# tiborcamargo/KinectPy

Hardware: AMD Instinct MI355X
Metric: Mpoints/sec end-to-end (unproject+filter+ICP), 4-sensor frame (higher is better)
Workload: dtype f64 decisions / f32 storage

## Files before the change

### kinectpy_amd/csrc/kpx_icpdefs.h

```cpp
#pragma once
#include <limits.h>

#include "kpx_internal.h"

namespace kpx {

typedef double d4 __attribute__((ext_vector_type(4)));
#ifndef KPX_ICP_WPE
#define KPX_ICP_WPE 3
#endif

#ifndef KPX_ICP_WAVES
#define KPX_ICP_WAVES 4
#endif
constexpr int kIWaves = KPX_ICP_WAVES;
constexpr int kIThreads = kIWaves * 64;
constexpr int kRT = 2;
constexpr int kWaves = 4;
constexpr int kRowsPerBlock = kWaves * kRT * 16;
constexpr int kCT = 32;
constexpr int kStageDoubles = kCT * 64;
#ifndef KPX_SEED_STRIDE
#define KPX_SEED_STRIDE 128
#endif
constexpr int kSeedStride = KPX_SEED_STRIDE;
constexpr double kSentinel = 1e300;
constexpr int kFRT = 4;
constexpr int kFRowsPerBlock = kWaves * kFRT * 16;
constexpr int kFCT = 64;
constexpr int kFStageFloats = kFCT * 64;
constexpr int kCand = 64;
constexpr int kAcc = 44;

struct IcpState {
    double T[16];
    double fitness, rmse;
    double count;
    int32_t iter, done;
    double motion, reach;
    double last_motion;
    double smax;
};
// ... 53 lines not shown
        int slot = 17;
#pragma unroll
        for (int a = 0; a < 6; ++a)
#pragma unroll
            for (int c = a; c < 6; ++c) put(slot++, J[a] * J[c]);
#pragma unroll
        for (int a = 0; a < 6; ++a) put(38 + a, J[a] * res);
    }
}
__host__ __device__ __forceinline__ unsigned long long progress_searched(unsigned long long searched, int64_t n)
{
    const unsigned long long cls = n > 0 ? (searched * 127ull + (unsigned long long)n - 1ull) / (unsigned long long)n : 0ull;
    return (cls > 127ull ? 127ull : cls) << 33;
}
constexpr int kSearchedWord = 8;
__device__ __forceinline__ unsigned long long searched_take(unsigned long long *ticket, int lane_in_block)
{
    unsigned long long v = 0ull;
    if (lane_in_block < 8) {
        v = __hip_atomic_load(ticket + kSearchedWord + lane_in_block, __ATOMIC_RELAXED, __HIP_MEMORY_SCOPE_AGENT);
        __hip_atomic_store(ticket + kSearchedWord + lane_in_block, 0ull, __ATOMIC_RELAXED, __HIP_MEMORY_SCOPE_AGENT);
    }
    if (lane_in_block < 64) {
        unsigned lo = (unsigned)v, hi = (unsigned)(v >> 32);
#pragma unroll
        for (int o = 1; o < 8; o <<= 1) {
            const unsigned ol = (unsigned)__shfl_xor((int)lo, o, 64), oh = (unsigned)__shfl_xor((int)hi, o, 64);
            const unsigned long long sum = (((unsigned long long)hi << 32) | lo) + (((unsigned long long)oh << 32) | ol);
            lo = (unsigned)sum; hi = (unsigned)(sum >> 32);
        }
        v = ((unsigned long long)hi << 32) | lo;
    }
    return v;
}
__device__ __forceinline__ double tile_tree16(const double *x)
{
    double a[8];
#pragma unroll
    for (int i = 0; i < 8; ++i) a[i] = x[2 * i] + x[2 * i + 1];
    return ((a[0] + a[1]) + (a[2] + a[3])) + ((a[4] + a[5]) + (a[6] + a[7]));
}
typedef unsigned u2 __attribute__((ext_vector_type(2)));
__device__ __forceinline__ unsigned hi32(double v) { return __builtin_bit_cast(u2, v)[1]; }

struct RobustLoss {
    int32_t kind;
    double k;
    __device__ __forceinline__ double weight(double r) const
    {
        switch (kind) {
        case KPX_LOSS_L1: return 1.0 / fabs(r);
        case KPX_LOSS_HUBER: return k / fmax(fabs(r), k);
        case KPX_LOSS_CAUCHY: { const double q = r / k; return 1.0 / (1.0 + q * q); }
        case KPX_LOSS_GM: { const double d = k + r * r; return k / (d * d); }
        case KPX_LOSS_TUKEY: { const double q = fmin(1.0, fabs(r) / k); const double u = 1.0 - q * q; return u * u; }
        default: return 1.0;
        }
    }
};
__device__ __forceinline__ void robust_row(const RobustLoss &loss, const double J[6], double r, double *acc)
{
    const double w = loss.weight(r);
    if (!isfinite(w)) return;
    double wJ[6];
#pragma unroll
    for (int p = 0; p < 6; ++p) wJ[p] = w * J[p];
    int q = 17;
#pragma unroll
    for (int p = 0; p < 6; ++p)
#pragma unroll
        for (int c = p; c < 6; ++c) acc[q++] += wJ[p] * J[c];
#pragma unroll
    for (int p = 0; p < 6; ++p) acc[38 + p] += wJ[p] * r;
// ... 82 lines not shown
```

### kinectpy_amd/csrc/kpx_icpiter.h

```cpp
#pragma once
#include "kpx_icpdefs.h"
#include "kpx_fixed.h"
#include "kpx_icpsolve.h"
#include "kpx_nnlocal.h"

namespace kpx {

constexpr int kIRows = kIWaves * kLRows;
constexpr int kCertHist = 64;
constexpr int kChainRec = 32;
constexpr int kChainRecords = 64;
constexpr int kChainWords = 24;
constexpr unsigned long long kChainEmpty = 0xFFF8C0DEC0DEC0DEull;
constexpr int kAccSet = kAccCopies * kAcc * kFixedWords;
constexpr int kStampBlocks = 4096;
__device__ unsigned long long g_icp_stamp[kStampBlocks][8];
__device__ unsigned long long g_icp_wave[kStampBlocks * 4][4];
__device__ unsigned long long g_cert_check[8];
__device__ unsigned long long g_chain_stamp[64][48];
__device__ __forceinline__ void chain_tick(unsigned long long *row, int slot, bool on)
{
    if (row && on) row[slot] = wall_clock64();
}
__device__ __forceinline__ void phase_tick(unsigned long long *__restrict__ armed, int slot, unsigned bid)
// ... 55 lines not shown
    if (first && g_cert_check[2] == 0ull) {
        g_cert_check[3] = (unsigned long long)k; g_cert_check[4] = __builtin_bit_cast(unsigned long long, st->last_motion);
        g_cert_check[5] = __builtin_bit_cast(unsigned long long, st->motion); g_cert_check[6] = __builtin_bit_cast(unsigned long long, c_skin);
    }
    atomicAdd(&g_cert_check[0], (unsigned long long)certified);
    atomicAdd(&g_cert_check[1], (unsigned long long)searched);
}
__device__ __forceinline__ IcpFuse ticket_fuse(const IcpProblem &P, int max_iter, double rel_fit, double rel_rmse, unsigned long long tag, int light,
                                               CertPolicy pol, double *chain_rec, unsigned long long *stamp)
{
    return IcpFuse{ (IcpState *)nullptr, P.ring, max_iter, rel_fit, rel_rmse, P.result, P.progress, tag, P.ring + kAccSet,
                    (light & 1) ? P.light_key : (double *)nullptr, P.sbbox, (light & 2) ? P.cert : (uint32_t *)nullptr,
                    (light & 2) ? P.thist : (double *)nullptr, (light & 4) ? 1 : 0, pol, chain_rec, stamp };
}
template <int THREADS, bool SEARCHED>
__device__ __forceinline__ unsigned long long winner_take(unsigned long long *acc, unsigned long long *ticket, int nacc, double *s_sums, int tix_w)
{
    if (tix_w < kAcc) s_sums[tix_w] = tix_w < nacc ? fixed_total_coherent(acc, tix_w) : 0.0;
    const unsigned long long n_searched = SEARCHED ? searched_take(ticket, tix_w) : 0ull;
    if (THREADS > 64) __syncthreads(); else wave_lds_fence();
    for (int e = tix_w; e < kAccSet; e += THREADS) __hip_atomic_store(acc + e, 0ull, __ATOMIC_RELAXED, __HIP_MEMORY_SCOPE_AGENT);
    if (tix_w == 0) __hip_atomic_store(ticket, 0ull, __ATOMIC_RELAXED, __HIP_MEMORY_SCOPE_AGENT);
    return n_searched;
}
__device__ __forceinline__ void winner_publish(IcpState *st, const IcpState *work, double *thist, int k, unsigned long long *progress, unsigned long long tag,
                                               unsigned long long n_searched, int64_t n, int lane)
{
    if (lane < (int)(sizeof(IcpState) / sizeof(double))) reinterpret_cast<double *>(st)[lane] = reinterpret_cast<const double *>(work)[lane];
    if (thist && k + 1 < kCertHist && lane < 12) thist[12 * (k + 1) + lane] = work->T[lane];
    if (lane == 0 && progress)
        __hip_atomic_store(progress, tag | progress_searched(n_searched, n) | ((unsigned long long)(work->done ? 1 : 0) << 32) | (unsigned long long)(unsigned)(k + 1),
                           __ATOMIC_RELAXED, __HIP_MEMORY_SCOPE_SYSTEM);
}

template <bool PERSIST = false>
__device__ __forceinline__ void icp_iter_body(const unsigned bid, const unsigned nblocks, const float *__restrict__ src, int64_t n, const float *__restrict__ tgt,
                                                       const float *__restrict__ tn, const double *__restrict__ Bs,
                                                       const int32_t *__restrict__ orig, const float *__restrict__ tile_box,
                                                       const float *__restrict__ group_box, int32_t n_groups,
                                                       const double *__restrict__ tbbox, const int32_t *__restrict__ row_of,
                                                       const float *__restrict__ src_sorted, int32_t *__restrict__ idx_sorted,
                                                       float *__restrict__ ptgt_sorted,
                                                       int32_t *__restrict__ idx_cur, double *__restrict__ d2_cur, double max_d2, int mode,
                                                       int k, const IcpState *__restrict__ st, unsigned long long *acc,
                                                       unsigned long long *__restrict__ tile_visits, IcpFuse fuse)
{
    const unsigned tix = PERSIST ? (unsigned)opaque_i((int)threadIdx.x) : threadIdx.x;
    __shared__ IcpState s_state;
    __shared__ double s_sums[kAcc];
    __shared__ float rowk[kIWaves][16][8];
    __shared__ float rowsrc[kIWaves][16][3];
    __shared__ uint32_t rowc[kIWaves][16];
    __shared__ int32_t rowi[kIWaves][16][2];
    __shared__ double s_key;
    const int wave = PERSIST ? __builtin_amdgcn_readfirstlane((int)(tix >> 6)) : (int)(tix >> 6), lane = tix & 63, q = lane >> 4, j = lane & 15;
    const int64_t row_base = ((int64_t)bid * kIWaves + wave) * kLRows;
    const int64_t last = n - 1;
    const unsigned long long t_block_start = (tile_visits && tix == 0) ? wall_clock64() : 0ull;
    const double t2max = target_t2max(tbbox);
    float my_src[3] = { 0.0f, 0.0f, 0.0f }, my_pt[3] = { 0.0f, 0.0f, 0.0f }, my_nrm[3] = { 0.0f, 0.0f, 0.0f };
    int32_t my_row = 0, my_prev = -1;
    uint32_t my_cert = 0u;
    const bool certs = fuse.ticket && fuse.light_key && fuse.cert;
    if (PERSIST && k > 0) {
        if (lane < 16) {
            my_row = rowi[wave][lane][1];
#pragma unroll
            for (int a = 0; a < 3; ++a) { my_src[a] = rowsrc[wave][lane][a]; my_pt[a] = rowk[wave][lane][a]; my_nrm[a] = rowk[wave][lane][3 + a]; }
            my_prev = __float_as_int(rowk[wave][lane][6]);
            if (certs) my_cert = rowc[wave][lane];
        }
    } else if (lane < 16) {
        const int64_t r = row_base + lane < last ? row_base + lane : last;
        if (idx_cur || d2_cur) my_row = row_of[r];
#pragma unroll
        for (int a = 0; a < 3; ++a) my_src[a] = src_sorted[3 * r + a];
        if (PERSIST) {
#pragma unroll
            for (int a = 0; a < 3; ++a) rowsrc[wave][lane][a] = my_src[a];
            rowc[wave][lane] = 0u;
        }
        if (k > 0) {
            my_prev = idx_sorted[r];
#pragma unroll
            for (int a = 0; a < 3; ++a) my_pt[a] = ptgt_sorted[3 * r + a];
            if (certs) my_cert = fuse.cert[r];
        }
    }
    __shared__ double s_thist[kCertHist][12];
    if (PERSIST) {
        if (certs && k < kCertHist && tix < 12) s_thist[k][tix] = st->T[tix];
    } else if (certs && k > 0)
        for (int e = tix; e < 12 * (k < kCertHist ? k : kCertHist); e += kIThreads) (&s_thist[0][0])[e] = fuse.thist[e];
    GroupPre gpre;
    group_pre_load(gpre, group_box, n_groups, lane);
    if (!PERSIST && mode == 1 && k > 0 && lane < 16) {
        const float *np_ = tn + 3 * (int64_t)(my_prev > 0 ? my_prev : 0);
#pragma unroll
        for (int a = 0; a < 3; ++a) my_nrm[a] = np_[a];
    }
    const double *Tk = st->T;
    static_assert(sizeof(IcpState) % sizeof(double) == 0, "IcpState is copied as doubles");
    if (fuse.ticket && tix < sizeof(IcpState) / sizeof(double))
        reinterpret_cast<double *>(&s_state)[tix] = reinterpret_cast<const double *>(st)[tix];
    if (fuse.pair) {
        const IcpState *in = fuse.pair + ((k + 1) & 1);
        IcpState *out = fuse.pair + (k & 1);
        const unsigned long long *prev = fuse.ring + (int64_t)((k + 2) % 3) * kAccSet;
        if (k > 0 && tix < kAcc) s_sums[tix] = (int)tix < (mode == 1 ? kAcc : 17) ? fixed_total(prev, tix) : 0.0;
        if (tix == 0) s_state = *in;
        __syncthreads();
        if (s_state.done) {
            if (bid == 0 && tix == 0) *out = s_state;
            return;
        }
        __shared__ FinishScratch s_fs;
        if (k > 0 && wave == 0)
            icp_finish_wave(s_sums, n, mode, k - 1, fuse.max_iter, fuse.rel_fit, fuse.rel_rmse, &s_state, bid == 0 ? fuse.result : (double *)nullptr,
                            s_fs, lane);
        __syncthreads();
        if (bid == 0) {
            unsigned long long *next = fuse.ring + (int64_t)((k + 1) % 3) * kAccSet;
            for (int e = tix; e < kAccSet; e += kIThreads) next[e] = 0ull;
            if (tix == 0) {
                *out = s_state;
                if (k > 0 && fuse.progress)
                    __hip_atomic_store(fuse.progress, fuse.tag | ((unsigned long long)(s_state.done ? 1 : 0) << 32) | (unsigned long long)(unsigned)k,
                                       __ATOMIC_RELEASE, __HIP_MEMORY_SCOPE_SYSTEM);
            }
        }
        if (s_state.done) return;
        Tk = s_state.T;
        acc = fuse.ring + (int64_t)(k % 3) * kAccSet;
    } else if (st->done) return;
    bool skip = false;
    if (fuse.ticket && fuse.light_key) {
        const double key = PERSIST ? (k > 0 ? s_key : 0.0) : fuse.light_key[bid];
        skip = key > 0.0 && (st->motion + st->reach) * (1.0 + 1e-6) + 1e-6 < key;
    }
    __shared__ double s_light[kIWaves];
    const int nacc = mode == 1 ? kAcc : 17;
    if (tile_visits && tix == 0 && bid < kStampBlocks) { g_icp_stamp[bid][7] = skip ? 1ull : 0ull; g_icp_stamp[bid][6] = (unsigned long long)nblocks; }
    do {
    if (skip) break;
    __shared__ int32_t lists[kIWaves][kLScratch];
    __shared__ double rowd[kIWaves][16][kRowStride];
    __shared__ float rowf[kIWaves][16][kRowFStride];
    __shared__ double sh[kAcc][kIRows + 1];
    if (tile_visits && tix == 0 && bid < kStampBlocks) {
        g_icp_stamp[bid][0] = t_block_start;
        g_icp_stamp[bid][6] = (unsigned long long)nblocks;
    }
    phase_tick(tile_visits, 1, bid);
    if (certs && (k > 0 || PERSIST)) __syncthreads();
    if (PERSIST && fuse.stamp && tix == 0) {
        const unsigned long long t = wall_clock64();
        if (bid == 0) fuse.stamp[0] = t;
        atomicMax(&fuse.stamp[5], t);
        atomicMin(&fuse.stamp[10], t);
    }

    const double c_reach = certs ? st->reach : 0.0;
    const double c_skin = cert_skin(certs, k, st, max_d2, fuse.pol);
    bool my_active = true, my_certd = false;
    if (lane < 16) {
        const int64_t i = my_row;
        double s[3];
        xform_row(Tk, my_src, s);
        const double seed = row_seed(s);
        double bv = INFINITY;
        int32_t bj = INT_MAX;
        if (k > 0 && my_prev >= 0) { bv = partner_bound(s, seed, my_pt); bj = my_prev; }
        bound_clamp(seed, max_d2, t2max, bv, bj);
        double rb0 = bv - 1.0;
        if (certs) {
            const bool certd = cert_test(s, my_src, my_prev, my_pt, bj, my_cert, s_thist[my_cert & 63u], c_reach, c_skin, fuse.cert_check, rb0);
            my_active = (!certd || fuse.cert_check) && row_base + lane <= last;
            my_certd = certd && row_base + lane <= last;
        }
        rowd[wave][lane][0] = s[0]; rowd[wave][lane][1] = s[1]; rowd[wave][lane][2] = s[2];
        rowd[wave][lane][3] = rb0;
        rowd[wave][lane][4] = seed; rowd[wave][lane][5] = bv;
        rowi[wave][lane][0] = bj; rowi[wave][lane][1] = (int32_t)i;
#pragma unroll
        for (int a = 0; a < 3; ++a) { rowk[wave][lane][a] = my_pt[a]; rowk[wave][lane][3 + a] = my_nrm[a]; }
        rowk[wave][lane][6] = __int_as_float(my_prev);
    }
    if (PERSIST && fuse.stamp) {
        const bool searched = lane < 16 && my_active && !my_certd;
        const unsigned long long sm = __builtin_amdgcn_ballot_w64(searched);
        const unsigned long long np = __builtin_amdgcn_ballot_w64(searched && my_prev < 0);
        const unsigned long long nc = __builtin_amdgcn_ballot_w64(searched && (my_cert & ~63u) == 0u);
        if (lane == 0 && sm) {
            atomicAdd(&fuse.stamp[26], 1ull); atomicAdd(&fuse.stamp[27], (unsigned long long)__builtin_popcountll(sm));
            atomicAdd(&fuse.stamp[28], (unsigned long long)__builtin_popcountll(np)); atomicAdd(&fuse.stamp[29], (unsigned long long)__builtin_popcountll(nc));
        }
    }
    const unsigned act_mask = (unsigned)(__builtin_amdgcn_ballot_w64(lane < 16 && my_active) & 0xFFFFull);
    const unsigned certd_mask = (unsigned)(__builtin_amdgcn_ballot_w64(lane < 16 && my_certd) & 0xFFFFull);
    wave_lds_fence();
    WaveRows w;
    w.a = q < 3 ? rowd[wave][j][q] : 1.0;
    w.rows = &rowd[wave][0][0];
    w.rowsf = &rowf[wave][0][0];
#pragma unroll
    for (int r = 0; r < 4; ++r) {
        const int rr = q + 4 * r;
        w.seed[r] = rowd[wave][rr][4];
        w.best[r] = rowd[wave][rr][5];
        w.bcol[r] = rowi[wave][rr][0];
        w.rb0[r] = rowd[wave][rr][3];
    }
    w.skin = c_skin;
    w.act_mask = act_mask;
    w.light_gap2 = -1.0;
    w.dbg = (PERSIST && fuse.stamp && bid == 0 && wave == 0) ? fuse.stamp + 16 : (unsigned long long *)nullptr;
    phase_tick(tile_visits, 2, bid);
    if (PERSIST) chain_tick(fuse.stamp, 1, bid == 0 && tix == 0);
    const unsigned long long t_sweep = tile_visits ? wall_clock64() : 0ull;
    unsigned long long swept = 0ull;
    int lane_p = 0, wave_p = 0, q_p = 0, j_p = 0;
    int64_t row_base_p = 0;
    auto rederive = [&]() {
        lane_p = opaque_i((int)(threadIdx.x & 63)); wave_p = opaque_i((int)(threadIdx.x >> 6)); q_p = lane_p >> 4; j_p = lane_p & 15;
        row_base_p = ((int64_t)bid * kIWaves + wave_p) * kLRows;
    };
    if (act_mask != 0u) {
        wave_lds_fence();
        swept = sweep_wave<true, true, PERSIST>(w, Bs, orig, tile_box, group_box, n_groups, t2max, lists[wave], &gpre);
        rederive();
        if (certs && fuse.cert_check && j_p == 0) {
#pragma unroll
            for (int r = 0; r < 4; ++r) {
                const int rr = q_p + 4 * r;
                if (((certd_mask >> rr) & 1u) != 0u && w.bcol[r] != rowi[wave_p][rr][0])
                    cert_check_disagreement(k, row_base_p + rr, rowi[wave_p][rr][0], w.bcol[r], PERSIST ? rowc[wave_p][rr] : fuse.cert[row_base_p + rr]);
            }
        }
        if (certs && j_p == 0) {
#pragma unroll
            for (int r = 0; r < 4; ++r) {
                const int rr = q_p + 4 * r;
                if (((act_mask >> rr) & 1u) != 0u && ((certd_mask >> rr) & 1u) == 0u) {
                    const uint32_t cw = cert_word(w.sec[r], w.eps_out, w.rb_out[r], k);
                    if (PERSIST) rowc[wave_p][rr] = cw; else fuse.cert[row_base_p + rr] = cw;
                }
            }
        }
    }
    if (act_mask == 0u) rederive();
    __shared__ int s_cnt[kIWaves];
    if (lane_p == 0) s_cnt[wave_p] = __builtin_popcount(act_mask & ~certd_mask);
    const unsigned visited = (unsigned)(swept & 0xFFFFu);
    if (certs && fuse.cert_check && lane_p == 0)
        cert_check_count(bid == 0 && wave_p == 0, k, st, c_skin, __builtin_popcount(certd_mask), __builtin_popcount(act_mask & ~certd_mask));
    if (lane_p == 0) s_light[wave_p] = act_mask == 0xFFFFu ? w.light_gap2 : -1.0;
    if (tile_visits && lane_p == 0 && bid < kStampBlocks && kIWaves <= 4) {
        unsigned long long *o = g_icp_wave[bid * 4 + wave_p];
        int with = 0;
#pragma unroll
        for (int r = 0; r < 4; ++r) with += (w.bcol[r] >= 0 && w.bcol[r] != INT_MAX) ? 1 : 0;
        o[0] = t_sweep; o[1] = wall_clock64(); o[2] = swept; o[3] = (unsigned long long)with;
    }
    phase_tick(tile_visits, 3, bid);
    if (PERSIST) chain_tick(fuse.stamp, 2, bid == 0 && lane_p == 0 && wave_p == 0);
    if (PERSIST && fuse.stamp && bid == 0 && lane_p == 0 && wave_p == 0) { fuse.stamp[13] = swept; fuse.stamp[14] = (unsigned long long)act_mask | ((unsigned long long)certd_mask << 16); }
    if (tile_visits && lane_p == 0) atomicAdd(tile_visits + ((bid * kIWaves + wave_p) & (kVisitSlots - 1)), (unsigned long long)visited);
    wave_lds_fence();
    if (j_p == 0) {
#pragma unroll
        for (int r = 0; r < 4; ++r) rowi[wave_p][q_p + 4 * r][0] = w.bcol[r];
    }
    wave_lds_fence();

    const int lane_e = lane_p, wave_e = wave_p;
    if (lane_e < 16) {
        const int col = wave_e * 16 + lane_e;
        for (int a = 0; a < nacc; ++a) sh[a][col] = 0.0;
        if (row_base_p + lane_e <= last) {
            const int32_t bj = rowi[wave_e][lane_e][0];
            const int64_t i = rowi[wave_e][lane_e][1];
            const bool none = bj < 0 || bj == INT_MAX;
            const int32_t out_j = none ? -1 : bj;
            const int32_t prev_j = __float_as_int(rowk[wave_e][lane_e][6]);
            const bool changed = k == 0 || out_j != prev_j;
            if (idx_cur) idx_cur[i] = out_j;
            if (PERSIST) rowk[wave_e][lane_e][6] = __int_as_float(out_j);
            else if (changed) idx_sorted[row_base_p + lane_e] = out_j;
            if (none) {
                if (d2_cur) d2_cur[i] = INFINITY;
            } else {
                const double s[3] = { rowd[wave_e][lane_e][0], rowd[wave_e][lane_e][1], rowd[wave_e][lane_e][2] };
                float tf[3] = { rowk[wave_e][lane_e][0], rowk[wave_e][lane_e][1], rowk[wave_e][lane_e][2] }, nf[3] = { rowk[wave_e][lane_e][3], rowk[wave_e][lane_e][4], rowk[wave_e][lane_e][5] };
                if (changed) {
                    const float *tp = tgt + 3 * (int64_t)bj;
#pragma unroll
                    for (int c = 0; c < 3; ++c) tf[c] = tp[c];
                    if (mode == 1) {
                        const float *np_ = tn + 3 * (int64_t)bj;
#pragma unroll
                        for (int c = 0; c < 3; ++c) nf[c] = np_[c];
                    }
#pragma unroll
                    for (int c = 0; c < 3; ++c) {
                        if (PERSIST) { rowk[wave_e][lane_e][c] = tf[c]; rowk[wave_e][lane_e][3 + c] = nf[c]; }
                        else ptgt_sorted[3 * (row_base_p + lane_e) + c] = tf[c];
                    }
                }
                const double t[3] = { (double)tf[0], (double)tf[1], (double)tf[2] };
                const double d2 = pair_d2(s, t);
                if (d2_cur) d2_cur[i] = d2;
                if (d2 < max_d2) pair_terms(s, t, d2, mode == 1, nf, [&](int slot, double v) { sh[slot][col] = v; });
            }
        }
    }
    __syncthreads();
    phase_tick(tile_visits, 4, bid);
    const int tix_e = wave_e * 64 + lane_e;
    if (tix_e < nacc) {
        unsigned long long lo = 0ull, hi = 0ull;
#pragma unroll
        for (int t = 0; t < kIWaves; ++t) {
            unsigned long long l, h;
            fixed_split(tile_tree16(&sh[tix_e][16 * t]), l, h);
            fixed_accumulate(lo, hi, l, h);
        }
        unsigned long long *slot = acc + (((int64_t)(bid & (kAccCopies - 1)) * kAcc + tix_e) * kFixedWords);
        if (fuse.ticket) fixed_add_words_performed(slot, lo, hi); else fixed_add_words(slot, lo, hi);
    } else if (!PERSIST && fuse.ticket && tix_e == nacc) {
        int cnt = 0;
#pragma unroll
        for (int wv = 0; wv < kIWaves; ++wv) cnt += s_cnt[wv];
        if (cnt) {
            const unsigned long long back = __hip_atomic_fetch_add(fuse.ticket + kSearchedWord + (bid & 7u), (unsigned long long)cnt, __ATOMIC_RELAXED, __HIP_MEMORY_SCOPE_AGENT);
            asm volatile("" ::"v"(back));
        }
    }
    if (fuse.light_key && tix == kIThreads - 1) {
        double g2 = INFINITY;
        bool light = true;
#pragma unroll
        for (int wv = 0; wv < kIWaves; ++wv) { light = light && s_light[wv] >= 0.0; g2 = fmin(g2, s_light[wv]); }
        const double nk = light ? st->motion + sqrt(g2) * (1.0 - 1e-9) : 0.0;
        if (PERSIST) s_key = nk; else fuse.light_key[bid] = nk;
    }
    phase_tick(tile_visits, 5, bid);
    } while (false);
    if (PERSIST && fuse.stamp && tix == 0) {
        const unsigned long long t = wall_clock64();
        if (bid == 0) fuse.stamp[3] = t;
        atomicMax(&fuse.stamp[11], t);
    }
    if (!fuse.ticket) return;
    __shared__ unsigned s_ticket;
    __syncthreads();
    if (tix == 0) s_ticket = (unsigned)__hip_atomic_fetch_add(fuse.ticket, 1ull, __ATOMIC_RELAXED, __HIP_MEMORY_SCOPE_AGENT);
    __syncthreads();
// ... 16 lines not shown
    const double *tbbox_w = tbbox;
    asm volatile("" : "+s"(tbbox_w));
    const double t2max_w = target_t2max(tbbox_w);
    IcpState *stw = const_cast<IcpState *>(st);
    IcpState *work = &s_state;
    if (PERSIST)
        icp_finish_wave_call(s_sums, n, mode, k, fuse.max_iter, fuse.rel_fit, fuse.rel_rmse, work, (double *)nullptr, &s_tail, lane,
                             fuse.light_key ? fuse.sbbox : (const double *)nullptr, max_d2, t2max_w, fuse.stamp ? fuse.stamp + 32 : (unsigned long long *)nullptr);
    else
        icp_finish_wave(s_sums, n, mode, k, fuse.max_iter, fuse.rel_fit, fuse.rel_rmse, work, fuse.result, s_tail, lane,
                        LightSkip{ fuse.light_key ? fuse.sbbox : (const double *)nullptr, max_d2, t2max_w });
    wave_lds_fence();
    if (PERSIST) chain_tick(fuse.stamp, 8, lane == 0);
    if (PERSIST) {
        static_assert(sizeof(IcpState) == kChainWords * sizeof(double), "record layout");
        __syncthreads();
        if (lane < kChainWords)
            __hip_atomic_store(reinterpret_cast<unsigned long long *>(fuse.chain_rec + (size_t)kChainRec * (k + 1)) + lane,
                               reinterpret_cast<const unsigned long long *>(&s_state)[lane], __ATOMIC_RELAXED, __HIP_MEMORY_SCOPE_AGENT);
        if (work->done && fuse.result) {
            if (lane < 16) fuse.result[lane] = work->T[lane];
            if (lane == 0) { fuse.result[16] = work->fitness; fuse.result[17] = work->rmse; fuse.result[18] = (double)k; fuse.result[19] = work->count; }
        }
        if (lane == 0 && fuse.progress && work->done)
            __hip_atomic_store(fuse.progress, fuse.tag | (1ull << 32) | (unsigned long long)(unsigned)(k + 1), __ATOMIC_RELAXED, __HIP_MEMORY_SCOPE_SYSTEM);
        chain_tick(fuse.stamp, 9, lane == 0);
        if (fuse.stamp && lane == 0) fuse.stamp[12] = __builtin_amdgcn_s_memtime();
        return;
    }
    winner_publish(stw, work, fuse.cert ? fuse.thist : (double *)nullptr, k, fuse.progress, fuse.tag, n_searched, n, lane);
}


__global__ __launch_bounds__(kIThreads) __attribute__((amdgpu_waves_per_eu(KPX_ICP_WPE, KPX_ICP_WPE))) void icp_iter_kernel(const float *__restrict__ src, int64_t n, const float *__restrict__ tgt,
                                                       const float *__restrict__ tn, const double *__restrict__ Bs,
                                                       const int32_t *__restrict__ orig, const float *__restrict__ tile_box,
                                                       const float *__restrict__ group_box, int32_t n_groups,
                                                       const double *__restrict__ tbbox, const int32_t *__restrict__ row_of,
                                                       const float *__restrict__ src_sorted, int32_t *__restrict__ idx_sorted,
                                                       float *__restrict__ ptgt_sorted,
                                                       int32_t *__restrict__ idx_cur, double *__restrict__ d2_cur, double max_d2, int mode,
                                                       int k, const IcpState *__restrict__ st, unsigned long long *acc,
                                                       unsigned long long *__restrict__ tile_visits, IcpFuse fuse)
{
    icp_iter_body(blockIdx.x, gridDim.x, src, n, tgt, tn, Bs, orig, tile_box, group_box, n_groups, tbbox, row_of, src_sorted, idx_sorted, ptgt_sorted,
                  idx_cur, d2_cur, max_d2, mode, k, st, acc, tile_visits, fuse);
}

__global__ __launch_bounds__(kIThreads) __attribute__((amdgpu_waves_per_eu(KPX_ICP_WPE, KPX_ICP_WPE))) void icp_iter_batch_kernel(IcpBatchArgs args, double max_d2, int mode, int max_iter, double rel_fit,
                                                       double rel_rmse, unsigned long long *__restrict__ tile_visits, int light, CertPolicy pol)
{
    const IcpProblem &P = args.p[batch_problem(args)];
    const unsigned bid = blockIdx.x - P.block0;
    const float *__restrict__ tgt = P.tgt, *__restrict__ tn = P.tn, *__restrict__ tile_box = P.tile_box, *__restrict__ group_box = P.group_box;
    const double *__restrict__ Bs = P.Bs, *__restrict__ tbbox = P.tbbox;
    const int32_t *__restrict__ orig = P.orig;
    const int32_t n_groups = P.n_groups;
    const int k = P.k;
    const IcpFuse fuse = ticket_fuse(P, max_iter, rel_fit, rel_rmse, P.tag, light, pol, nullptr, nullptr);
    icp_iter_body(bid, P.blocks, P.src, P.n, tgt, tn, Bs, orig, tile_box, group_box, n_groups, tbbox, P.row_of, P.src_sorted, P.idx_sorted, P.ptgt_sorted,
                  P.idx_cur, P.d2_cur, max_d2, mode, k, P.pair, P.ring, tile_visits, fuse);
}

__global__ __launch_bounds__(kIThreads) __attribute__((amdgpu_waves_per_eu(KPX_ICP_WPE, KPX_ICP_WPE))) void icp_chain_kernel(IcpBatchArgs args, const float *__restrict__ tgt,
                                                       const float *__restrict__ tn, const double *__restrict__ Bs,
                                                       const int32_t *__restrict__ orig, const float *__restrict__ tile_box,
                                                       const float *__restrict__ group_box, int32_t n_groups,
                                                       const double *__restrict__ tbbox, double max_d2, int mode, int max_iter, double rel_fit,
                                                       double rel_rmse, unsigned long long tag, unsigned long long *__restrict__ tile_visits, int light,
                                                       CertPolicy pol, unsigned long long limit_ticks, unsigned long long *abort_word)
{
    const int pi = batch_problem(args);
    const IcpProblem &P = args.p[pi];
    const unsigned bid = blockIdx.x - P.block0;
    __shared__ IcpState s_cur;
    __shared__ int s_abort;
    const unsigned long long t0 = wall_clock64();
    if (threadIdx.x == 0) s_abort = 0;
    __syncthreads();
    for (int k = 0; k <= max_iter; ++k) {
        asm volatile("" : "+s"(tgt), "+s"(tn), "+s"(Bs), "+s"(orig), "+s"(tile_box), "+s"(group_box), "+s"(tbbox));
        asm volatile("" : "+s"(max_d2), "+s"(mode), "+s"(n_groups), "+s"(pol.calm), "+s"(pol.factor), "+s"(pol.smin), "+s"(pol.smax));
// ... 57 lines not shown
```

### kinectpy_amd/csrc/kpx_icprows.h

```cpp
#pragma once
#include "kpx_icpiter.h"

namespace kpx {

constexpr int kRowsBlock = 64;
static_assert(kRowsBlock == kIRows, "IcpProblem::block0 / blocks count 64-row blocks for icp_iter_batch_kernel and icp_rows_kernel alike");

constexpr int kDppXor1 = 0xB1, kDppXor2 = 0x4E, kDppHalfMirror = 0x141, kDppMirror = 0x140;
__device__ __forceinline__ double row16_tree_sum(double v)
{
    v += dpp_f64<kDppXor1>(v);
    v += dpp_f64<kDppXor2>(v);
    v += dpp_f64<kDppHalfMirror>(v);
    v += dpp_f64<kDppMirror>(v);
    return v;
}

template <int MODE>
__global__ __launch_bounds__(64) __attribute__((amdgpu_waves_per_eu(KPX_ICP_WPE, KPX_ICP_WPE))) void icp_rows_kernel(IcpBatchArgs args, double max_d2, int max_iter, double rel_fit,
                                                                                                                     double rel_rmse, unsigned long long *__restrict__ tile_visits,
                                                                                                                     int light, CertPolicy pol)
{
    constexpr int NACC = MODE == 1 ? kAcc : 17;
    const IcpProblem P = args.p[batch_problem(args)];
    const unsigned bid = blockIdx.x - P.block0;
    const int k = P.k;
    IcpState *const st = P.pair;
    if (st->done) return;

    __shared__ IcpState s_state;
    __shared__ double s_sums[kAcc];
    __shared__ FinishScratch s_tail;
    __shared__ double rowd[kRowsBlock][kRowStride];
    __shared__ float rowf[kLRows][kRowFStride];
    __shared__ float rowk[kRowsBlock][11];
    __shared__ int32_t rowi[kRowsBlock];
    __shared__ uint32_t rowc[kRowsBlock];
    __shared__ int32_t rowm[kRowsBlock];
    __shared__ int32_t lists[kLScratch];
    static_assert(kLScratch * sizeof(int32_t) >= 4 * kAcc * sizeof(double), "the tile partials reuse the sweep's scratch");
    double (*s_part)[kAcc] = reinterpret_cast<double (*)[kAcc]>(lists);

    const int lane = threadIdx.x;
    const unsigned long long lt = (1ull << lane) - 1ull;
    const int64_t last = P.n - 1;
    const int64_t row = (int64_t)bid * kRowsBlock + lane;
    const bool valid = lane < kRowsBlock && row <= last;
    const int64_t r = valid ? row : last;
    const bool certs = (light & 2) != 0, use_light = (light & 1) != 0, cert_check = (light & 4) != 0;
// ... 217 lines not shown
```

### kinectpy_amd/csrc/kpx_nnlocal.h

```cpp
#pragma once
#include "kpx_icpdefs.h"
#include "kpx_morton.h"

namespace kpx {

constexpr int kLGroupTiles = 16;
constexpr int kLRows = 16;
constexpr int kLList = 320;
constexpr int kVisitSlots = 1024;

__global__ __launch_bounds__(256) void nn_local_prep_kernel(const float *__restrict__ tgt, int64_t m, double *__restrict__ Bs,
                                                            int32_t *__restrict__ orig, float *__restrict__ tile_box,
                                                            float *__restrict__ group_box)
{
    const int64_t j = (int64_t)blockIdx.x * 256 + threadIdx.x;
    double b0 = 0.0, b1 = 0.0, b2 = 0.0, b3 = kSentinel;
    float lo[3] = { kBoxBig, kBoxBig, kBoxBig }, hi[3] = { -kBoxBig, -kBoxBig, -kBoxBig };
    if (j < m) {
        const int64_t o = orig[j];
        const float fx = tgt[3 * o], fy = tgt[3 * o + 1], fz = tgt[3 * o + 2];
        const double tx = fx, ty = fy, tz = fz;
        b0 = -2.0 * tx; b1 = -2.0 * ty; b2 = -2.0 * tz;
        b3 = fma(tx, tx, fma(ty, ty, tz * tz));
        lo[0] = hi[0] = fx; lo[1] = hi[1] = fy; lo[2] = hi[2] = fz;
// ... 43 lines not shown
    if (r >= n) return;
    const int64_t i = row_of[r];
    double s[3];
    xform_row(T, src + 3 * i, s);
    const double seed = row_seed(s);
    reinterpret_cast<double2 *>(A64)[2 * r] = make_double2(s[0], s[1]);
    reinterpret_cast<double2 *>(A64)[2 * r + 1] = make_double2(s[2], 1.0);
    K64[r] = seed;
    double bv = INFINITY;
    int32_t bj = INT_MAX;
    if (prev) {
        const int32_t j = prev[i];
        if (j >= 0 && j != INT_MAX) { bv = partner_bound(s, seed, tgt + 3 * (int64_t)j); bj = j; }
    }
    if (max_d2 > 0.0) bound_clamp(seed, max_d2, target_t2max(tbbox), bv, bj);
    init_val[r] = bv;
    init_idx[r] = bj;
}

__device__ __forceinline__ unsigned fold16(unsigned long long m) { return (unsigned)((m | (m >> 16) | (m >> 32) | (m >> 48)) & 0xFFFFull); }

template <int CTRL>
__device__ __forceinline__ int dpp_i32(int v) { return __builtin_amdgcn_update_dpp(v, v, CTRL, 0xF, 0xF, false); }
template <int CTRL>
__device__ __forceinline__ double dpp_f64(double v)
{
    typedef int i2 __attribute__((ext_vector_type(2)));
    i2 b = __builtin_bit_cast(i2, v);
    b[0] = dpp_i32<CTRL>(b[0]);
    b[1] = dpp_i32<CTRL>(b[1]);
    return __builtin_bit_cast(double, b);
}
constexpr int kRor1 = 0x121, kRor2 = 0x122, kRor4 = 0x124, kRor8 = 0x128;
__device__ __forceinline__ double row16_all_max(double v)
{
    v = fmax(v, dpp_f64<kRor1>(v)); v = fmax(v, dpp_f64<kRor2>(v)); v = fmax(v, dpp_f64<kRor4>(v)); v = fmax(v, dpp_f64<kRor8>(v));
    return v;
}
__device__ __forceinline__ double row16_all_min(double v)
{
    v = fmin(v, dpp_f64<kRor1>(v)); v = fmin(v, dpp_f64<kRor2>(v)); v = fmin(v, dpp_f64<kRor4>(v)); v = fmin(v, dpp_f64<kRor8>(v));
    return v;
}
__device__ __forceinline__ double readlane_f64(double v, int l)
{
    typedef int i2 __attribute__((ext_vector_type(2)));
    i2 b = __builtin_bit_cast(i2, v);
    b[0] = __builtin_amdgcn_readlane(b[0], l);
    b[1] = __builtin_amdgcn_readlane(b[1], l);
    return __builtin_bit_cast(double, b);
}
__device__ __forceinline__ double wave_uniform_max(double v)
{
    v = row16_all_max(v);
    return fmax(fmax(readlane_f64(v, 0), readlane_f64(v, 16)), fmax(readlane_f64(v, 32), readlane_f64(v, 48)));
}

__device__ __forceinline__ double quad_uniform_max(double v)
{
    return fmax(fmax(readlane_f64(v, 0), readlane_f64(v, 16)), fmax(readlane_f64(v, 32), readlane_f64(v, 48)));
}

__device__ __forceinline__ float f32_down(double x)
{
    float f = (float)x;
    if ((double)f > x) f = f > 0.0f ? __int_as_float(__float_as_int(f) - 1) : (f < 0.0f ? __int_as_float(__float_as_int(f) + 1) : -1.401298464e-45f);
// ... 45 lines not shown
constexpr int kGroupPre = 2;
struct GroupPre {
    float b[kGroupPre][6];
};
__device__ __forceinline__ void group_box_load(float b[6], const float *__restrict__ group_box, int32_t n_groups, int gi)
{
    const bool on = gi < n_groups;
    const float *bx = group_box + (int64_t)(on ? gi : 0) * 6;
#pragma unroll
    for (int a = 0; a < 3; ++a) { b[a] = on ? bx[a] : kBoxBig; b[3 + a] = on ? bx[3 + a] : -kBoxBig; }
}
__device__ __forceinline__ void group_pre_load(GroupPre &g, const float *__restrict__ group_box, int32_t n_groups, int lane)
{
#pragma unroll
    for (int t = 0; t < kGroupPre; ++t) group_box_load(g.b[t], group_box, n_groups, 64 * t + lane);
}
__device__ __forceinline__ double box_gap2v(const double slo[3], const double shi[3], const float bx[6])
{
    double g2 = 0.0;
#pragma unroll
    for (int a = 0; a < 3; ++a) {
        const double g = fmax(0.0, fmax((double)bx[a] - shi[a], slo[a] - (double)bx[3 + a]));
        g2 = fma(g, g, g2);
    }
    return g2;
}

__device__ __forceinline__ double wave_uniform_min(double v)
{
    v = row16_all_min(v);
    return fmin(fmin(readlane_f64(v, 0), readlane_f64(v, 16)), fmin(readlane_f64(v, 32), readlane_f64(v, 48)));
}

template <bool PRE, bool CERT = false, bool LOOPED = false>
__device__ __forceinline__ unsigned long long sweep_wave(WaveRows &w, const double *__restrict__ Bs, const int32_t *__restrict__ orig,
                                                         const float *__restrict__ tile_box, const float *__restrict__ group_box,
                                                         int32_t n_groups, const double t2max, int32_t *scr, const GroupPre *pre)
{
    const int lane = LOOPED ? opaque_i((int)(threadIdx.x & 63)) : (int)(threadIdx.x & 63), q = lane >> 4, j = lane & 15;
    const unsigned long long lt = (1ull << lane) - 1ull;
    auto dbg_tick = [&](int slot) { if (LOOPED && w.dbg && lane == 0) w.dbg[slot] = wall_clock64(); };
    dbg_tick(0);
    int32_t *list = scr, *cand = scr + kLList, *surv = scr + kLList + 7 * kLCand;
    double *const rowq = w.rows + kRowStride * q;
    float *const rowfq = w.rowsf + kRowFStride * q;
    constexpr double kRel = 1.0 + 9.31322574615478515625e-10;
    double slo[3], shi[3];
    {
        const bool act_j = !CERT || ((w.act_mask >> j) & 1u) != 0u;
        const double mn = row16_all_min(act_j ? w.a : INFINITY), mx = row16_all_max(act_j ? w.a : -INFINITY);
#pragma unroll
        for (int k = 0; k < 3; ++k) { slo[k] = readlane_f64(mn, 16 * k); shi[k] = readlane_f64(mx, 16 * k); }
    }
    const double kmax = quad_uniform_max(fmax(fmax(w.seed[0], w.seed[1]), fmax(w.seed[2], w.seed[3])));
    const double eps = ldexp(kmax + t2max + 1.0, -38);
    double rb[4];
#pragma unroll
    for (int r = 0; r < 4; ++r) rb[r] = (CERT ? w.rb0[r] : w.best[r] - 1.0) * kRel + eps;
    if (CERT) {
#pragma unroll
        for (int r = 0; r < 4; ++r) w.sec[r] = 0xFFFFFFFFu;
    }
    double R2 = quad_uniform_max(fmax(fmax(rb[0], rb[1]), fmax(rb[2], rb[3])));
    if (!(R2 < 1e290)) {
        double u[4] = { INFINITY, INFINITY, INFINITY, INFINITY };
        for (int g0 = 0; g0 < n_groups; g0 += 16) {
            const int g = g0 + j;
// ... 4 lines not shown
                for (int r = 0; r < 4; ++r) {
                    const double *pr = w.rows + kRowStride * (q + 4 * r);
                    u[r] = fmin(u[r], pt_far2(pr[0], pr[1], pr[2], lo, hi));
                }
            }
        }
#pragma unroll
        for (int r = 0; r < 4; ++r) rb[r] = fmin(rb[r], row16_all_min(u[r]) * kRel + eps);
        R2 = quad_uniform_max(fmax(fmax(rb[0], rb[1]), fmax(rb[2], rb[3])));
    }
    auto publish_bounds = [&](const double rbv[4]) {
        if (j == 0) {
#pragma unroll
            for (int r = 0; r < 4; ++r) {
                rowq[4 * kRowStride * r + kRowBound] = rbv[r];
                rowfq[4 * kRowFStride * r + kRowFBound] = f32_up(rbv[r]);
            }
        }
    };
    if (q < 3) {
        w.rowsf[kRowFStride * j + q] = f32_down(w.a);
        w.rowsf[kRowFStride * j + 3 + q] = f32_up(w.a);
    }
    publish_bounds(rb);
    dbg_tick(1);

    const double bpad = q == 3 ? kSentinel : 0.0;
    int nlist = 0, ns = 0;
    unsigned visited = 0, box_trips = 0, mul_trips = 0, groups_kept = 0;

    auto multiply = [&]() {
        wave_lds_fence();
        bool updated = false;
        for (int e0 = 0; e0 < nlist; e0 += kMulBatch) {
            double b[kMulBatch];
            int32_t oc[kMulBatch];
#pragma unroll
            for (int h = 0; h < kMulBatch; ++h) {
                const int32_t t = e0 + h < nlist ? list[e0 + h] : -1;
                b[h] = t >= 0 ? Bs[(int64_t)t * 64 + lane] : bpad;
                oc[h] = t >= 0 ? orig[(int64_t)t * 16 + j] : INT_MAX;
            }
            ++mul_trips;
            if (mul_trips == 1) dbg_tick(5);
#pragma unroll
            for (int h0 = 0; h0 < kMulBatch; h0 += 4) {
                if (e0 + h0 >= nlist) break;
                const d4 c0 = __builtin_amdgcn_mfma_f64_16x16x4f64(w.a, b[h0], w.seed, 0, 0, 0);
                const d4 c1 = __builtin_amdgcn_mfma_f64_16x16x4f64(w.a, b[h0 + 1], w.seed, 0, 0, 0);
                const d4 c2 = __builtin_amdgcn_mfma_f64_16x16x4f64(w.a, b[h0 + 2], w.seed, 0, 0, 0);
                const d4 c3 = __builtin_amdgcn_mfma_f64_16x16x4f64(w.a, b[h0 + 3], w.seed, 0, 0, 0);
#define KPX_NNL_TILE(ACC, COL)                                                                      \
                {                                                                                   \
                    bool pass = false;                                                              \
                    _Pragma("unroll") for (int r = 0; r < 4; ++r) pass |= hi32(ACC[r]) <= hi32(w.best[r]); \
                    if (__builtin_amdgcn_ballot_w64(pass) != 0) {                                   \
                        updated = true;                                                             \
                        _Pragma("unroll") for (int r = 0; r < 4; ++r) {                            \
                            const bool tk = (int)(ACC[r] < w.best[r]) | ((int)(ACC[r] == w.best[r]) & (int)((COL) < w.bcol[r])); \
                            if (CERT) {      \
                                const unsigned lose = tk ? hi32(w.best[r]) : ((COL) == w.bcol[r] ? 0xFFFFFFFFu : hi32(ACC[r])); \
                                w.sec[r] = lose < w.sec[r] ? lose : w.sec[r];                       \
                            }                                                                       \
                            w.best[r] = tk ? ACC[r] : w.best[r];                                   \
                            w.bcol[r] = tk ? (COL) : w.bcol[r];                                    \
                        }                                                                           \
                    } else if (CERT) {       \
                        _Pragma("unroll") for (int r = 0; r < 4; ++r) w.sec[r] = hi32(ACC[r]) < w.sec[r] ? hi32(ACC[r]) : w.sec[r]; \
                    }                                                                               \
                }
                KPX_NNL_TILE(c0, oc[h0]) KPX_NNL_TILE(c1, oc[h0 + 1]) KPX_NNL_TILE(c2, oc[h0 + 2]) KPX_NNL_TILE(c3, oc[h0 + 3])
#undef KPX_NNL_TILE
            }
        }
        if (mul_trips <= 2) dbg_tick(6);
        visited += (unsigned)nlist;
        nlist = 0;
        bool gain = false;
        auto next_bound = [&](int r) {
            double nb = w.best[r] - 1.0;
            if (CERT && w.skin > 0.0) {
                const double rr = (double)(sqrtf(f32_up(fmax(nb, 0.0))) * 1.0000002384185791015625f) + w.skin;
                nb = fmax(nb, rr * rr);
            }
            return nb;
        };
        if (updated) {
#pragma unroll
            for (int r = 0; r < 4; ++r) gain |= next_bound(r) < kTightenGain * (double)rowfq[4 * kRowFStride * r + kRowFBound];
        }
        if (updated && __builtin_amdgcn_ballot_w64(gain) != 0) {
            double nrb[4];
#pragma unroll
            for (int r = 0; r < 4; ++r) nrb[r] = fmin(rowq[4 * kRowStride * r + kRowBound], row16_all_min(next_bound(r)) * kRel + eps);
            R2 = quad_uniform_max(fmax(fmax(nrb[0], nrb[1]), fmax(nrb[2], nrb[3])));
            wave_lds_fence();
            publish_bounds(nrb);
        }
        wave_lds_fence();
        dbg_tick(7);
    };

    auto tiles_of_survivors = [&]() {
        wave_lds_fence();
// ... 206 lines not shown
```

Measured before the change: 2515.

## Reduce ICP tile partials in registers via DPP and drop shared accumulator array

Replaces the per-block shared accumulator array (kAcc x rows) with a wave-level reduction. Each lane computes a quarter of the accumulator slots, sums them across 16 rows with DPP tree sums, and writes the partials into the wave's existing sweep scratch. Certificate transform history is also loaded per lane from global memory in the non-persistent path, which removes an extra block barrier. The MFMA grouping and multiply batch are parameterized for the block kernel, with separate waves-per-EU knobs. This cuts LDS usage and synchronization, at the cost of redundant pair-term computation across lanes and more register pressure.

After: 2524, median of 6. About the same (+0.4%).

```diff
diff --git a/kinectpy_amd/csrc/kpx_icpdefs.h b/kinectpy_amd/csrc/kpx_icpdefs.h
--- a/kinectpy_amd/csrc/kpx_icpdefs.h
+++ b/kinectpy_amd/csrc/kpx_icpdefs.h
@@ -8,6 +8,9 @@
 typedef double d4 __attribute__((ext_vector_type(4)));
 #ifndef KPX_ICP_WPE
 #define KPX_ICP_WPE 3
+#endif
+#ifndef KPX_ICP_BLOCK_WPE
+#define KPX_ICP_BLOCK_WPE 3
 #endif
 
 #ifndef KPX_ICP_WAVES
@@ -127,13 +130,6 @@
         v = ((unsigned long long)hi << 32) | lo;
     }
     return v;
-}
-__device__ __forceinline__ double tile_tree16(const double *x)
-{
-    double a[8];
-#pragma unroll
-    for (int i = 0; i < 8; ++i) a[i] = x[2 * i] + x[2 * i + 1];
-    return ((a[0] + a[1]) + (a[2] + a[3])) + ((a[4] + a[5]) + (a[6] + a[7]));
 }
 typedef unsigned u2 __attribute__((ext_vector_type(2)));
 __device__ __forceinline__ unsigned hi32(double v) { return __builtin_bit_cast(u2, v)[1]; }
diff --git a/kinectpy_amd/csrc/kpx_icpiter.h b/kinectpy_amd/csrc/kpx_icpiter.h
--- a/kinectpy_amd/csrc/kpx_icpiter.h
+++ b/kinectpy_amd/csrc/kpx_icpiter.h
@@ -111,6 +111,39 @@
         __hip_atomic_store(progress, tag | progress_searched(n_searched, n) | ((unsigned long long)(work->done ? 1 : 0) << 32) | (unsigned long long)(unsigned)(k + 1),
                            __ATOMIC_RELAXED, __HIP_MEMORY_SCOPE_SYSTEM);
 }
+
+__device__ __forceinline__ double (*chain_thist())[12]
+{
+    __shared__ double s_thist[kCertHist][12];
+    return s_thist;
+}
+template <int G>
+__device__ __forceinline__ void pair_quad_partials(bool in, const double s[3], const double t[3], double d2, bool plane, const float *nrm, int q, bool writer,
+                                                   double *part)
+{
+    static_assert(4 * G <= kAcc, "part[] holds kAcc doubles");
+    double c[G];
+#pragma unroll
+    for (int a = 0; a < G; ++a) c[a] = 0.0;
+    const int qq = in ? q : -1;
+    pair_terms(s, t, d2, plane, nrm, [&](int slot, double v) { c[slot % G] = slot / G == qq ? v : c[slot % G]; });
+#pragma unroll
+    for (int a = 0; a < G; ++a) c[a] = row16_tree_sum(c[a]);
+    if (writer) {
+#pragma unroll
+        for (int a = 0; a < G; ++a) part[G * q + a] = c[a];
+    }
+}
+#ifndef KPX_ICP_BLOCK_MUL_BATCH
+#define KPX_ICP_BLOCK_MUL_BATCH KPX_MUL_BATCH
+#endif
+constexpr int kIBlockMulBatch = KPX_ICP_BLOCK_MUL_BATCH;
+#ifndef KPX_ICP_BLOCK_MFMA_GROUP
+#define KPX_ICP_BLOCK_MFMA_GROUP 4
+#endif
+constexpr int kIBlockMfmaGroup = KPX_ICP_BLOCK_MFMA_GROUP;
+static_assert(kIBlockMfmaGroup == 1 || kIBlockMfmaGroup == 2 || kIBlockMfmaGroup == 4, "MGRP divides the four tiles of a step");
+static_assert(kIBlockMulBatch >= 4 && kIBlockMulBatch % 4 == 0, "the multiply loop consumes its batch four tiles at a time");
 
 template <bool PERSIST = false>
 __device__ __forceinline__ void icp_iter_body(const unsigned bid, const unsigned nblocks, const float *__restrict__ src, int64_t n, const float *__restrict__ tgt,
@@ -166,13 +199,19 @@
             if (certs) my_cert = fuse.cert[r];
         }
     }
-    __shared__ double s_thist[kCertHist][12];
-    if (PERSIST) {
-        if (certs && k < kCertHist && tix < 12) s_thist[k][tix] = st->T[tix];
-    } else if (certs && k > 0)
-        for (int e = tix; e < 12 * (k < kCertHist ? k : kCertHist); e += kIThreads) (&s_thist[0][0])[e] = fuse.thist[e];
+    double my_th[12];
+#pragma unroll
+    for (int e = 0; e < 12; ++e) my_th[e] = 0.0;
+    if constexpr (PERSIST) {
+        if (certs && k < kCertHist && tix < 12) chain_thist()[k][tix] = st->T[tix];
+    }
     GroupPre gpre;
     group_pre_load(gpre, group_box, n_groups, lane);
+    if (!PERSIST && certs && k > 0 && lane < 16 && __uint_as_float(my_cert & ~63u) > 0.0f) {
+        const double *th = fuse.thist + 12 * (int)(my_cert & 63u);
+#pragma unroll
+        for (int e = 0; e < 12; ++e) my_th[e] = th[e];
+    }
     if (!PERSIST && mode == 1 && k > 0 && lane < 16) {
         const float *np_ = tn + 3 * (int64_t)(my_prev > 0 ? my_prev : 0);
 #pragma unroll
@@ -222,16 +261,16 @@
     if (tile_visits && tix == 0 && bid < kStampBlocks) { g_icp_stamp[bid][7] = skip ? 1ull : 0ull; g_icp_stamp[bid][6] = (unsigned long long)nblocks; }
     do {
     if (skip) break;
-    __shared__ int32_t lists[kIWaves][kLScratch];
+    __shared__ __attribute__((aligned(8))) int32_t lists[kIWaves][kLScratch];
+    static_assert(kLScratch % 2 == 0 && kLScratch * sizeof(int32_t) >= kAcc * sizeof(double), "a wave's tile partial reuses its sweep scratch");
     __shared__ double rowd[kIWaves][16][kRowStride];
     __shared__ float rowf[kIWaves][16][kRowFStride];
-    __shared__ double sh[kAcc][kIRows + 1];
     if (tile_visits && tix == 0 && bid < kStampBlocks) {
         g_icp_stamp[bid][0] = t_block_start;
         g_icp_stamp[bid][6] = (unsigned long long)nblocks;
     }
     phase_tick(tile_visits, 1, bid);
-    if (certs && (k > 0 || PERSIST)) __syncthreads();
+    if (PERSIST && certs) __syncthreads();
     if (PERSIST && fuse.stamp && tix == 0) {
         const unsigned long long t = wall_clock64();
         if (bid == 0) fuse.stamp[0] = t;
@@ -253,7 +292,9 @@
         bound_clamp(seed, max_d2, t2max, bv, bj);
         double rb0 = bv - 1.0;
         if (certs) {
-            const bool certd = cert_test(s, my_src, my_prev, my_pt, bj, my_cert, s_thist[my_cert & 63u], c_reach, c_skin, fuse.cert_check, rb0);
+            const double *Th = my_th;
+            if constexpr (PERSIST) Th = chain_thist()[my_cert & 63u];
+            const bool certd = cert_test(s, my_src, my_prev, my_pt, bj, my_cert, Th, c_reach, c_skin, fuse.cert_check, rb0);
             my_active = (!certd || fuse.cert_check) && row_base + lane <= last;
             my_certd = certd && row_base + lane <= last;
         }
@@ -306,7 +347,7 @@
     };
     if (act_mask != 0u) {
         wave_lds_fence();
-        swept = sweep_wave<true, true, PERSIST>(w, Bs, orig, tile_box, group_box, n_groups, t2max, lists[wave], &gpre);
+        swept = sweep_wave<true, true, PERSIST, PERSIST ? kMulBatch : kIBlockMulBatch, PERSIST ? 4 : kIBlockMfmaGroup>(w, Bs, orig, tile_box, group_box, n_groups, t2max, lists[wave], &gpre);
         rederive();
         if (certs && fuse.cert_check && j_p == 0) {
 #pragma unroll
@@ -354,8 +395,6 @@
 
     const int lane_e = lane_p, wave_e = wave_p;
     if (lane_e < 16) {
-        const int col = wave_e * 16 + lane_e;
-        for (int a = 0; a < nacc; ++a) sh[a][col] = 0.0;
         if (row_base_p + lane_e <= last) {
             const int32_t bj = rowi[wave_e][lane_e][0];
             const int64_t i = rowi[wave_e][lane_e][1];
@@ -382,16 +421,28 @@
                     }
 #pragma unroll
                     for (int c = 0; c < 3; ++c) {
-                        if (PERSIST) { rowk[wave_e][lane_e][c] = tf[c]; rowk[wave_e][lane_e][3 + c] = nf[c]; }
-                        else ptgt_sorted[3 * (row_base_p + lane_e) + c] = tf[c];
+                        rowk[wave_e][lane_e][c] = tf[c]; rowk[wave_e][lane_e][3 + c] = nf[c];
+                        if (!PERSIST) ptgt_sorted[3 * (row_base_p + lane_e) + c] = tf[c];
                     }
                 }
                 const double t[3] = { (double)tf[0], (double)tf[1], (double)tf[2] };
                 const double d2 = pair_d2(s, t);
                 if (d2_cur) d2_cur[i] = d2;
-                if (d2 < max_d2) pair_terms(s, t, d2, mode == 1, nf, [&](int slot, double v) { sh[slot][col] = v; });
             }
         }
+    }
+    wave_lds_fence();
+    {
+        const int j_e = lane_e & 15, q_e = lane_e >> 4;
+        const int32_t bj = rowi[wave_e][j_e][0];
+        const double s[3] = { rowd[wave_e][j_e][0], rowd[wave_e][j_e][1], rowd[wave_e][j_e][2] };
+        const double t[3] = { (double)rowk[wave_e][j_e][0], (double)rowk[wave_e][j_e][1], (double)rowk[wave_e][j_e][2] };
+        const float nf[3] = { rowk[wave_e][j_e][3], rowk[wave_e][j_e][4], rowk[wave_e][j_e][5] };
+        const double d2 = pair_d2(s, t);
+        const bool in = row_base_p + j_e <= last && bj >= 0 && bj != INT_MAX && d2 < max_d2;
+        double *const part = reinterpret_cast<double *>(lists[wave_e]);
+        if (mode == 1) pair_quad_partials<(kAcc + 3) / 4>(in, s, t, d2, true, nf, q_e, j_e == 0, part);
+        else pair_quad_partials<(17 + 3) / 4>(in, s, t, d2, false, nf, q_e, j_e == 0, part);
     }
     __syncthreads();
     phase_tick(tile_visits, 4, bid);
@@ -401,7 +452,7 @@
 #pragma unroll
         for (int t = 0; t < kIWaves; ++t) {
             unsigned long long l, h;
-            fixed_split(tile_tree16(&sh[tix_e][16 * t]), l, h);
+            fixed_split(reinterpret_cast<const double *>(lists[t])[tix_e], l, h);
             fixed_accumulate(lo, hi, l, h);
         }
         unsigned long long *slot = acc + (((int64_t)(bid & (kAccCopies - 1)) * kAcc + tix_e) * kFixedWords);
@@ -484,7 +535,7 @@
 }
 
 
-__global__ __launch_bounds__(kIThreads) __attribute__((amdgpu_waves_per_eu(KPX_ICP_WPE, KPX_ICP_WPE))) void icp_iter_kernel(const float *__restrict__ src, int64_t n, const float *__restrict__ tgt,
+__global__ __launch_bounds__(kIThreads) __attribute__((amdgpu_waves_per_eu(KPX_ICP_BLOCK_WPE, KPX_ICP_BLOCK_WPE))) void icp_iter_kernel(const float *__restrict__ src, int64_t n, const float *__restrict__ tgt,
                                                        const float *__restrict__ tn, const double *__restrict__ Bs,
                                                        const int32_t *__restrict__ orig, const float *__restrict__ tile_box,
                                                        const float *__restrict__ group_box, int32_t n_groups,
@@ -499,7 +550,7 @@
                   idx_cur, d2_cur, max_d2, mode, k, st, acc, tile_visits, fuse);
 }
 
-__global__ __launch_bounds__(kIThreads) __attribute__((amdgpu_waves_per_eu(KPX_ICP_WPE, KPX_ICP_WPE))) void icp_iter_batch_kernel(IcpBatchArgs args, double max_d2, int mode, int max_iter, double rel_fit,
+__global__ __launch_bounds__(kIThreads) __attribute__((amdgpu_waves_per_eu(KPX_ICP_BLOCK_WPE, KPX_ICP_BLOCK_WPE))) void icp_iter_batch_kernel(IcpBatchArgs args, double max_d2, int mode, int max_iter, double rel_fit,
                                                        double rel_rmse, unsigned long long *__restrict__ tile_visits, int light, CertPolicy pol)
 {
     const IcpProblem &P = args.p[batch_problem(args)];
diff --git a/kinectpy_amd/csrc/kpx_icprows.h b/kinectpy_amd/csrc/kpx_icprows.h
--- a/kinectpy_amd/csrc/kpx_icprows.h
+++ b/kinectpy_amd/csrc/kpx_icprows.h
@@ -5,16 +5,6 @@
 
 constexpr int kRowsBlock = 64;
 static_assert(kRowsBlock == kIRows, "IcpProblem::block0 / blocks count 64-row blocks for icp_iter_batch_kernel and icp_rows_kernel alike");
-
-constexpr int kDppXor1 = 0xB1, kDppXor2 = 0x4E, kDppHalfMirror = 0x141, kDppMirror = 0x140;
-__device__ __forceinline__ double row16_tree_sum(double v)
-{
-    v += dpp_f64<kDppXor1>(v);
-    v += dpp_f64<kDppXor2>(v);
-    v += dpp_f64<kDppHalfMirror>(v);
-    v += dpp_f64<kDppMirror>(v);
-    return v;
-}
 
 template <int MODE>
 __global__ __launch_bounds__(64) __attribute__((amdgpu_waves_per_eu(KPX_ICP_WPE, KPX_ICP_WPE))) void icp_rows_kernel(IcpBatchArgs args, double max_d2, int max_iter, double rel_fit,
diff --git a/kinectpy_amd/csrc/kpx_nnlocal.h b/kinectpy_amd/csrc/kpx_nnlocal.h
--- a/kinectpy_amd/csrc/kpx_nnlocal.h
+++ b/kinectpy_amd/csrc/kpx_nnlocal.h
@@ -99,6 +99,15 @@
     return __builtin_bit_cast(double, b);
 }
 constexpr int kRor1 = 0x121, kRor2 = 0x122, kRor4 = 0x124, kRor8 = 0x128;
+constexpr int kDppXor1 = 0xB1, kDppXor2 = 0x4E, kDppHalfMirror = 0x141, kDppMirror = 0x140;
+__device__ __forceinline__ double row16_tree_sum(double v)
+{
+    v += dpp_f64<kDppXor1>(v);
+    v += dpp_f64<kDppXor2>(v);
+    v += dpp_f64<kDppHalfMirror>(v);
+    v += dpp_f64<kDppMirror>(v);
+    return v;
+}
 __device__ __forceinline__ double row16_all_max(double v)
 {
     v = fmax(v, dpp_f64<kRor1>(v)); v = fmax(v, dpp_f64<kRor2>(v)); v = fmax(v, dpp_f64<kRor4>(v)); v = fmax(v, dpp_f64<kRor8>(v));
@@ -210,7 +219,7 @@
     return fmin(fmin(readlane_f64(v, 0), readlane_f64(v, 16)), fmin(readlane_f64(v, 32), readlane_f64(v, 48)));
 }
 
-template <bool PRE, bool CERT = false, bool LOOPED = false>
+template <bool PRE, bool CERT = false, bool LOOPED = false, int MULB = kMulBatch, int MGRP = 4>
 __device__ __forceinline__ unsigned long long sweep_wave(WaveRows &w, const double *__restrict__ Bs, const int32_t *__restrict__ orig,
                                                          const float *__restrict__ tile_box, const float *__restrict__ group_box,
                                                          int32_t n_groups, const double t2max, int32_t *scr, const GroupPre *pre)
@@ -281,11 +290,11 @@
     auto multiply = [&]() {
         wave_lds_fence();
         bool updated = false;
-        for (int e0 = 0; e0 < nlist; e0 += kMulBatch) {
-            double b[kMulBatch];
-            int32_t oc[kMulBatch];
-#pragma unroll
-            for (int h = 0; h < kMulBatch; ++h) {
+        for (int e0 = 0; e0 < nlist; e0 += MULB) {
+            double b[MULB];
+            int32_t oc[MULB];
+#pragma unroll
+            for (int h = 0; h < MULB; ++h) {
                 const int32_t t = e0 + h < nlist ? list[e0 + h] : -1;
                 b[h] = t >= 0 ? Bs[(int64_t)t * 64 + lane] : bpad;
                 oc[h] = t >= 0 ? orig[(int64_t)t * 16 + j] : INT_MAX;
@@ -293,12 +302,11 @@
             ++mul_trips;
             if (mul_trips == 1) dbg_tick(5);
 #pragma unroll
-            for (int h0 = 0; h0 < kMulBatch; h0 += 4) {
+            for (int h0 = 0; h0 < MULB; h0 += 4) {
                 if (e0 + h0 >= nlist) break;
-                const d4 c0 = __builtin_amdgcn_mfma_f64_16x16x4f64(w.a, b[h0], w.seed, 0, 0, 0);
-                const d4 c1 = __builtin_amdgcn_mfma_f64_16x16x4f64(w.a, b[h0 + 1], w.seed, 0, 0, 0);
-                const d4 c2 = __builtin_amdgcn_mfma_f64_16x16x4f64(w.a, b[h0 + 2], w.seed, 0, 0, 0);
-                const d4 c3 = __builtin_amdgcn_mfma_f64_16x16x4f64(w.a, b[h0 + 3], w.seed, 0, 0, 0);
+                _Pragma("unroll") for (int h1 = h0; h1 < h0 + 4; h1 += MGRP) {
+                d4 c[MGRP];
+                _Pragma("unroll") for (int g = 0; g < MGRP; ++g) c[g] = __builtin_amdgcn_mfma_f64_16x16x4f64(w.a, b[h1 + g], w.seed, 0, 0, 0);
 #define KPX_NNL_TILE(ACC, COL)                                                                      \
                 {                                                                                   \
                     bool pass = false;                                                              \
@@ -318,7 +326,8 @@
                         _Pragma("unroll") for (int r = 0; r < 4; ++r) w.sec[r] = hi32(ACC[r]) < w.sec[r] ? hi32(ACC[r]) : w.sec[r]; \
                     }                                                                               \
                 }
-                KPX_NNL_TILE(c0, oc[h0]) KPX_NNL_TILE(c1, oc[h0 + 1]) KPX_NNL_TILE(c2, oc[h0 + 2]) KPX_NNL_TILE(c3, oc[h0 + 3])
+                _Pragma("unroll") for (int g = 0; g < MGRP; ++g) KPX_NNL_TILE(c[g], oc[h1 + g])
+                }
 #undef KPX_NNL_TILE
             }
         }
```
